# jontio/JAERO

Hardware: AMD Instinct MI355X
Metric: Msamples/s of real 48 kHz PCM through the 10.5 kbps OQPSK demodulator hot path (higher is better)
Workload: dtype f64; 1 GPU; 65536-channel-per-GPU synthetic 48 kHz 10.5 kbps OQPSK continuous (BASELINE configs[2] shape, scaled to 65536 channels per GPU = one wavefront of 64 channels per SIMD), 4096-sample writes, coarse 2^14 FFT every 4096 samples, AFC off, EbNo meters on, Eb/N0 10.0 dB, per-channel carrier (8000 +- 100 Hz), bits, noise, symbol phase; 42 untimed pre-roll steps (the last 11 resident and back to back with ; channels_per_gpu=65536, total_channels=65536, chunk=4096, ebno_meters=True, preroll_steps=42, timing_phases=32, hbm_bytes_per_resident_channel=2267392, resident_channels_max=136377, ranks=1, control_plane=none (single rank), sustain_steps=11

## Files before the change

jaero_amd/csrc/jaero_device.h:

```cpp
#pragma once
#include <hip/hip_runtime.h>
#include <stdint.h>
#include "jd_libm.h"

#define JD_WTSIZE 19999
#define JD_WAVE 64

enum
{
    S_M2_PTR, S_M2_STEP, S_M2_FREQ,
    S_MC_PTR, S_MC_STEP, S_MC_FREQ,
    S_ST_PTR, S_ST_STEP, S_ST_FREQ, S_ST_LAST,
    S_AGC_SUM,
    S_EB_ESUM, S_EB_E2SUM, S_EB_EBNO,
    S_D1,
    S_D41_1, S_D41_2, S_D41_3,
    S_D42_1, S_D42_2, S_D42_3,
    S_D8_1, S_D8_2,
    S_RES_X1, S_RES_X2, S_RES_Y1, S_RES_Y2,
    S_LF_X1, S_LF_X2, S_LF_Y1, S_LF_Y2,
    S_SIG2L_RE, S_SIG2L_IM, S_PTD_RE, S_PTD_IM,
    S_MARG_SUM, S_PM_SUM, S_MSEMA_SUM, S_MSE,
    S_DIFF_LAST,
    S_LOCKINGBW, S_THRESH,
    S_MFB_A0_RE, S_MFB_A0_IM,
    S_PRE_PTR, S_PRE_STEP, S_PRE_FSUM,
    S_PRE_PTR_NEXT, S_PRE_STEP_NEXT,
    S_NFIELDS
};
enum
{
    I_AGC_POS,
    I_AGC_HOLD,
    I_BB_PTR, I_COARSE_CNT,
    I_MARG_POS, I_DT_POS, I_PM_POS, I_MSEMA_POS,
    I_YUI, I_SIG2L_INIT, I_FLAGS, I_COUNTDOWN, I_COUNTDOWN2, I_EMPTYING, I_NEST,
    I_SOFT_CNT, I_SYM_CNT, I_LOG_CNT, I_OVERFLOW,
    I_DLY_POS,
    I_NFIELDS
};
typedef const __attribute__((address_space(4))) int jd_cint;
typedef const __attribute__((address_space(4))) double jd_cdouble;
__device__ __forceinline__ int jd_sload(const int *q) { return *(jd_cint *)q; }
__device__ __forceinline__ double jd_sload(const double *q) { return *(jd_cdouble *)q; }

#define JD_G4(row, ch, rows) ((((size_t)((ch) >> 2)) * (size_t)(rows) + (size_t)(row)) * 4 + (size_t)((ch) & 3))
#define LDF(f) (p.S[(size_t)(f) * nchp + ch])
#define LDI(f) (p.I[(size_t)(f) * nchp + ch])

#define JF_AFC 1
#define JF_SQL 2
#define JF_CPUREDUCE 4
#define JF_DCD 8

struct JGeom
{
    int kind, nch, nchp, ngroups;
    double Fs, fb;
    int Fs_int;
    int fir_n;
    int agc_len;
    int ebno_len;
    int win_len;
    int nfft, nfft_log2;
    int marg_len, dt_len, pm_len, msema_len;
    double ee;
    double w4, w8;
    int sps, sps2;
    double res_b0, res_b1, res_b2, res_a1, res_a2;
    double lf_b0, lf_b1, lf_b2, lf_a1, lf_a2;
    double stref_freq;
    double correctionfactor;
    unsigned flags;
    int soft_cap, sym_cap, log_cap;
};

struct JPtrs
{
    double *S;
    int *I;
    double *win;
    double2 *bbring;
    double *y;
    double *marg;
    double2 *dt;
    double *pm;
    double *msema;
    double *firsave;
    double2 *dly;
    double *dly8;
    int16_t *soft;
    double *sym;
    double *slog;
    const double2 *cis;
    const double *taps2;
    double *symrec;
};
#define JD_SYMREC_LEN 800

__device__ __forceinline__ int jd_cisidx(double wtptr)
{
    int t = (int)wtptr;
    if (t >= JD_WTSIZE) t = 0;
    if (t < 0) t = JD_WTSIZE - 1;
    return t;
}
__device__ __forceinline__ void jd_wt_next(double &ptr, double &step)
{
    if (step < 0) step = 0;
    ptr += step;
    while (((int)ptr) >= JD_WTSIZE) ptr -= JD_WTSIZE;
}
__device__ __forceinline__ void jd_wt_setfreq(double &freq, double &step, double f, double samplerate)
{
    freq = f;
    if (freq < 0) freq = 0;
    step = (freq) * ((double)JD_WTSIZE) / samplerate;
}
__device__ __forceinline__ void jd_wt_inc_phase_deg(double &ptr, double phase_deg)
{
    phase_deg += (360.0 * ptr / ((double)JD_WTSIZE));
    phase_deg = fmod(phase_deg, 360.0);
    while (phase_deg < 0) phase_deg += 360.0;
    ptr = (phase_deg / 360.0) * ((double)JD_WTSIZE);
}
__device__ __forceinline__ void jd_wt_advance_fraction(double &ptr, double f)
{
    ptr += f * JD_WTSIZE;
    while (ptr >= JD_WTSIZE) ptr -= JD_WTSIZE;
    while (ptr < 0) ptr += JD_WTSIZE;
}
__device__ __forceinline__ bool jd_wt_passed(double last_ptr, double ptr, double step, double fraction_of_wave, double &frac)
{
    double pt = (fraction_of_wave * JD_WTSIZE);
    double tl = last_ptr - pt;
    double tp = ptr - pt;
    if (tl < 0.0) tl += JD_WTSIZE;
    if (tp < 0.0) tp += JD_WTSIZE;
    if ((tl > (3.0 * JD_WTSIZE / 4.0)) && (tp < (1.0 * JD_WTSIZE / 4.0)))
    {
        frac = tp / step;
        return true;
    }
    return false;
}
__device__ __forceinline__ int jd_qround(double d)
{
    return d >= 0.0 ? (int)(d + 0.5) : (int)(d - (double)((int)(d - 1)) + 0.5) + (int)(d - 1);
}
__device__ __forceinline__ int jd_softbit(double v)
{
    int ibit = jd_qround(v);
    if (ibit > 255) ibit = 255;
    if (ibit < 0) ibit = 0;
    return ibit;
}

#define JD_EBNO_TAIL 192


template <int FIRN, int LDSN, int D, bool FUSED = false, int TAILA = 1>
__device__ __forceinline__ void jd_fir_eval(const double *lre, const double *lim, const double *ltap, const double (&tre)[TAILA],
                                            const double (&tim)[TAILA], int fir_slot, int lane, double &ore, double &oim)
{
    constexpr int TAILN = FIRN - LDSN;
    double pr[D], pi[D], pt[D];
    int slot = fir_slot;
    auto fetch = [&](int s, int q) {
        pt[q] = ltap[s];
        if (s >= TAILN)
        {
            pr[q] = lre[slot * 64 + lane];
            pi[q] = lim[slot * 64 + lane];
            slot++;
            if (slot >= LDSN) slot = 0;
        }
    };
#pragma unroll
    for (int s = 0; s < D; s++) fetch(s, s);
    __builtin_amdgcn_sched_barrier(0);
    double are = 0, aim = 0;
#pragma unroll
    for (int s = 0; s < FIRN; s++)
    {
        const int q = s % D;
        const double xr = (s < TAILN) ? tre[(TAILN - 1 - s) < 0 ? 0 : (TAILN - 1 - s)] : pr[q];
        const double xi = (s < TAILN) ? tim[(TAILN - 1 - s) < 0 ? 0 : (TAILN - 1 - s)] : pi[q];
        if constexpr (FUSED) { are = fma(pt[q], xr, are); aim = fma(pt[q], xi, aim); }
        else { are = are + pt[q] * xr; aim = aim + pt[q] * xi; }
        asm volatile("" : "+v"(are), "+v"(aim));
        if (s + D < FIRN) fetch(s + D, q);
        __builtin_amdgcn_sched_barrier(0);
    }
    ore = are; oim = aim;
}

struct JTaps28 { double t[28]; };

typedef __attribute__((address_space(3))) const double jd_lds_cdouble;
template <int FIRN, int LDSN, int D, int S, int TAP0, int NQ = LDSN>
__device__ __forceinline__ void jd_fir_lds_part(jd_lds_cdouble *lre_l, jd_lds_cdouble *lim_l, const JTaps28 &tp, double &are, double &aim)
{
    constexpr int TAILN = TAP0;
    double pr[D], pi[D];
#pragma unroll
    for (int q = 0; q < D; q++) { pr[q] = lre_l[((S + q) % LDSN) * 64]; pi[q] = lim_l[((S + q) % LDSN) * 64]; }
    __builtin_amdgcn_sched_barrier(0);
    auto tap_of = [&](int q) { const int s = TAILN + q; return tp.t[s <= 27 ? s : 54 - s]; };
    double mr = tap_of(0) * pr[0], mi = tap_of(0) * pi[0];
#pragma unroll
    for (int q = 0; q < NQ; q++)
    {
        double nr = 0, ni = 0;
        if (q + 1 < NQ) { nr = tap_of(q + 1) * pr[(q + 1) % D]; ni = tap_of(q + 1) * pi[(q + 1) % D]; }
        are = are + mr;
        aim = aim + mi;
        asm volatile("" : "+v"(are), "+v"(aim));
        if (q + D < NQ) { pr[q % D] = lre_l[((S + q + D) % LDSN) * 64]; pi[q % D] = lim_l[((S + q + D) % LDSN) * 64]; }
        mr = nr; mi = ni;
        __builtin_amdgcn_sched_barrier(0);
    }
}
template <int FIRN, int LDSN, int D, int TAILA>
__device__ __forceinline__ void jd_fir_eval_sym(const double *lre, const double *lim, const JTaps28 &tp, const double (&tre)[TAILA],
                                                const double (&tim)[TAILA], int fir_slot, int lane, double &ore, double &oim)
{
    static_assert(FIRN == 55, "symmetric-tap filter is the 55-tap RRC");
    constexpr int TAILN = FIRN - LDSN;
    double are = 0, aim = 0;
#pragma unroll
    for (int s = 0; s < TAILN; s++)
    {
        const double tap = tp.t[s <= 27 ? s : 54 - s];
        are = are + tap * tre[TAILN - 1 - s];
        aim = aim + tap * tim[TAILN - 1 - s];
    }
    int slot = fir_slot;
#pragma unroll 1
    for (int q = 0; q < LDSN; q++)
    {
        const int s = TAILN + q;
        const double tap = tp.t[s <= 27 ? s : 54 - s];
        are = are + tap * lre[slot * 64 + lane];
        aim = aim + tap * lim[slot * 64 + lane];
        slot++;
        if (slot >= LDSN) slot = 0;
    }
    ore = are; oim = aim;
}
template <int FIRN, int LDSN, int D, int TAILA>
__device__ __forceinline__ void jd_fir_eval_sym_static(const double *lre, const double *lim, const JTaps28 &tp, const double (&tre)[TAILA],
                                                       const double (&tim)[TAILA], int fir_slot, int lane, double &ore, double &oim)
{
    static_assert(FIRN == 55 && LDSN <= 40, "symmetric-tap filter is the 55-tap RRC; the switch below has 40 cases");
    constexpr int TAILN = FIRN - LDSN;
    jd_lds_cdouble *lre_l = (jd_lds_cdouble *)lre + lane, *lim_l = (jd_lds_cdouble *)lim + lane;
    double are = 0, aim = 0;
#pragma unroll
    for (int s = 0; s < TAILN; s++)
    {
        const double tap = tp.t[s <= 27 ? s : 54 - s];
        are = are + tap * tre[TAILN - 1 - s];
        aim = aim + tap * tim[TAILN - 1 - s];
    }
#define JD_FIR_CASE(S) case S: if constexpr (S < LDSN) jd_fir_lds_part<FIRN, LDSN, D, (S < LDSN ? S : 0), FIRN - LDSN>(lre_l, lim_l, tp, are, aim); break;
    switch (fir_slot)
    {
        JD_FIR_CASE(0) JD_FIR_CASE(1) JD_FIR_CASE(2) JD_FIR_CASE(3) JD_FIR_CASE(4) JD_FIR_CASE(5) JD_FIR_CASE(6) JD_FIR_CASE(7)
        JD_FIR_CASE(8) JD_FIR_CASE(9) JD_FIR_CASE(10) JD_FIR_CASE(11) JD_FIR_CASE(12) JD_FIR_CASE(13) JD_FIR_CASE(14) JD_FIR_CASE(15)
        JD_FIR_CASE(16) JD_FIR_CASE(17) JD_FIR_CASE(18) JD_FIR_CASE(19) JD_FIR_CASE(20) JD_FIR_CASE(21) JD_FIR_CASE(22) JD_FIR_CASE(23)
        JD_FIR_CASE(24) JD_FIR_CASE(25) JD_FIR_CASE(26) JD_FIR_CASE(27) JD_FIR_CASE(28) JD_FIR_CASE(29) JD_FIR_CASE(30) JD_FIR_CASE(31)
        JD_FIR_CASE(32) JD_FIR_CASE(33) JD_FIR_CASE(34) JD_FIR_CASE(35) JD_FIR_CASE(36) JD_FIR_CASE(37) JD_FIR_CASE(38) JD_FIR_CASE(39)
    default: break;
    }
#undef JD_FIR_CASE
    ore = are; oim = aim;
}

template <int FIRN, int LDSN, int D, int TAILA>
__device__ __forceinline__ void jd_fir_eval_sym_static_but_last(const double *lre, const double *lim, const JTaps28 &tp, const double (&tre)[TAILA],
                                                                const double (&tim)[TAILA], int slot_old, int lane, double &ore, double &oim)
{
    static_assert(FIRN == 55 && LDSN <= 40 && LDSN >= 8, "symmetric-tap filter is the 55-tap RRC; the switch below has 40 cases");
    constexpr int TAILN = FIRN - LDSN;
    jd_lds_cdouble *lre_l = (jd_lds_cdouble *)lre + lane, *lim_l = (jd_lds_cdouble *)lim + lane;
    double are = 0, aim = 0;
#pragma unroll
    for (int s = 0; s < TAILN; s++)
    {
        const double tap = tp.t[s <= 27 ? s : 54 - s];
        are = are + tap * tre[TAILN - 1 - s];
        aim = aim + tap * tim[TAILN - 1 - s];
    }
#define JD_FIR_CASE(S) case S: if constexpr (S < LDSN) jd_fir_lds_part<FIRN, LDSN, D, (S < LDSN ? (S + 1) % LDSN : 0), FIRN - LDSN, LDSN - 1>(lre_l, lim_l, tp, are, aim); break;
    switch (slot_old)
    {
        JD_FIR_CASE(0) JD_FIR_CASE(1) JD_FIR_CASE(2) JD_FIR_CASE(3) JD_FIR_CASE(4) JD_FIR_CASE(5) JD_FIR_CASE(6) JD_FIR_CASE(7)
        JD_FIR_CASE(8) JD_FIR_CASE(9) JD_FIR_CASE(10) JD_FIR_CASE(11) JD_FIR_CASE(12) JD_FIR_CASE(13) JD_FIR_CASE(14) JD_FIR_CASE(15)
        JD_FIR_CASE(16) JD_FIR_CASE(17) JD_FIR_CASE(18) JD_FIR_CASE(19) JD_FIR_CASE(20) JD_FIR_CASE(21) JD_FIR_CASE(22) JD_FIR_CASE(23)
        JD_FIR_CASE(24) JD_FIR_CASE(25) JD_FIR_CASE(26) JD_FIR_CASE(27) JD_FIR_CASE(28) JD_FIR_CASE(29) JD_FIR_CASE(30) JD_FIR_CASE(31)
        JD_FIR_CASE(32) JD_FIR_CASE(33) JD_FIR_CASE(34) JD_FIR_CASE(35) JD_FIR_CASE(36) JD_FIR_CASE(37) JD_FIR_CASE(38) JD_FIR_CASE(39)
    default: break;
    }
#undef JD_FIR_CASE
    ore = are; oim = aim;
}

__device__ __forceinline__ double jd_with_hi(double x, int h) { return __hiloint2double(h, __double2loint(x)); }
__device__ __forceinline__ double jd_expm1(double x)
{
    const double one = 1.0, huge = 1.0e+300, tiny = 1.0e-300, o_threshold = 7.09782712893383973096e+02,
                 ln2_hi = 6.93147180369123816490e-01, ln2_lo = 1.90821492927058770002e-10, invln2 = 1.44269504088896338700e+00,
                 Q1 = -3.33333333333331316428e-02, Q2 = 1.58730158725481460165e-03, Q3 = -7.93650757867487942473e-05,
                 Q4 = 4.00821782732936239552e-06, Q5 = -2.01099218183624371326e-07;
    double y, hi, lo, c = 0, t, e, hxs, hfx, r1;
    int k;
    unsigned hx = (unsigned)__double2hiint(x);
    const unsigned xsb = hx & 0x80000000u;
    hx &= 0x7fffffffu;
    if (hx >= 0x4043687Au)
    {
        if (hx >= 0x40862E42u)
        {
            if (hx >= 0x7ff00000u)
            {
                if (((hx & 0xfffffu) | (unsigned)__double2loint(x)) != 0) return x + x;
                return (xsb == 0) ? x : -1.0;
            }
            if (x > o_threshold) return huge * huge;
        }
        if (xsb != 0 && x + tiny < 0.0) return tiny - one;
    }
    if (hx > 0x3fd62e42u)
    {
        if (hx < 0x3FF0A2B2u)
        {
            if (xsb == 0) { hi = x - ln2_hi; lo = ln2_lo; k = 1; }
            else { hi = x + ln2_hi; lo = -ln2_lo; k = -1; }
        }
        else
        {
            k = (int)(invln2 * x + ((xsb == 0) ? 0.5 : -0.5));
            t = k;
            hi = x - t * ln2_hi;
            lo = t * ln2_lo;
        }
        x = hi - lo;
        c = (hi - x) - lo;
    }
    else if (hx < 0x3c900000u) return x;
    else k = 0;
    hfx = 0.5 * x;
    hxs = x * hfx;
    {
        const double R1 = one + hxs * Q1, h2 = hxs * hxs;
        const double R2 = Q2 + hxs * Q3, h4 = h2 * h2;
        const double R3 = Q4 + hxs * Q5;
        r1 = R1 + h2 * R2 + h4 * R3;
    }
    t = 3.0 - r1 * hfx;
    e = hxs * ((r1 - t) / (6.0 - x * t));
    if (k == 0) return x - (x * e - hxs);
    e = (x * (e - c) - c);
    e -= hxs;
    if (k == -1) return 0.5 * (x - e) - 0.5;
    if (k == 1)
    {
        if (x < -0.25) return -2.0 * (e - (x + 0.5));
        return one + 2.0 * (x - e);
    }
    if (k <= -2 || k > 56)
    {
        y = one - (e - x);
        y = jd_with_hi(y, __double2hiint(y) + (k << 20));
        return y - one;
    }
    if (k < 20)
    {
        t = jd_with_hi(one, 0x3ff00000 - (0x200000 >> k));
        y = t - (e - x);
        y = jd_with_hi(y, __double2hiint(y) + (k << 20));
    }
    else
    {
        t = jd_with_hi(one, (0x3ff - k) << 20);
        y = x - (e + t);
        y += one;
        y = jd_with_hi(y, __double2hiint(y) + (k << 20));
    }
    return y;
}
__device__ __noinline__ double jd_tanh_full(double x)
{
    const double one = 1.0, two = 2.0, tiny = 1.0e-300;
    double t, z;
    const int jx = __double2hiint(x);
    const int ix = jx & 0x7fffffff;
    if (ix >= 0x7ff00000) return (jx >= 0) ? one / x + one : one / x - one;
    if (ix < 0x40360000)
    {
        if ((ix | __double2loint(x)) == 0) return x;
        if (ix < 0x3c800000) return x * (one + x);
        const bool big = ix >= 0x3ff00000;
        const double ax2 = two * fabs(x);
        t = jd_expm1(big ? ax2 : -ax2);
        const double q = (big ? two : t) / (t + two);
        z = big ? one - q : -q;
    }
    else z = one - tiny;
    return (jx >= 0) ? z : -z;
}

__device__ __forceinline__ double jd_tanh(double xin)
{
    const double one = 1.0, two = 2.0, ln2_hi = 6.93147180369123816490e-01, ln2_lo = 1.90821492927058770002e-10,
                 invln2 = 1.44269504088896338700e+00, Q1 = -3.33333333333331316428e-02, Q2 = 1.58730158725481460165e-03,
                 Q3 = -7.93650757867487942473e-05, Q4 = 4.00821782732936239552e-06, Q5 = -2.01099218183624371326e-07;
    const int jx = __double2hiint(xin), ix = jx & 0x7fffffff;
    if (!(ix >= 0x3c800000 && ix < 0x401a0000)) return jd_tanh_full(xin);
    const bool big = ix >= 0x3ff00000;
    const double ax2 = two * fabs(xin);
    double x = big ? ax2 : -ax2;
    const unsigned hx = (unsigned)__double2hiint(x) & 0x7fffffffu;
    const int k = (hx > 0x3fd62e42u) ? (int)(invln2 * x + (big ? 0.5 : -0.5)) : 0;
    const double tk = (double)k;
    const double hi = x - tk * ln2_hi, lo = tk * ln2_lo;
    x = hi - lo;
    const double c = (hi - x) - lo;
    const double hfx = 0.5 * x, hxs = x * hfx;
    const double R1 = one + hxs * Q1, h2 = hxs * hxs, R2 = Q2 + hxs * Q3, h4 = h2 * h2, R3 = Q4 + hxs * Q5;
    const double r1 = R1 + h2 * R2 + h4 * R3;
    const double t3 = 3.0 - r1 * hfx;
    const double e = hxs * jd_div(r1 - t3, 6.0 - x * t3);
    const double r_k0 = x - (x * e - hxs);
    double e2 = (x * (e - c) - c);
    e2 -= hxs;
    const double r_m1 = 0.5 * (x - e2) - 0.5;
    double yn = one - (e2 - x);
    yn = jd_with_hi(yn, __double2hiint(yn) + (k << 20));
    const double r_neg = yn - one;
    const double tm = jd_with_hi(one, 0x3ff00000 - (0x200000 >> (k & 31)));
    double ym = tm - (e2 - x);
    ym = jd_with_hi(ym, __double2hiint(ym) + (k << 20));
    const double t = (k == 0) ? r_k0 : (k == -1) ? r_m1 : (k <= -2) ? r_neg : ym;
    const double q = jd_div(big ? two : t, t + two);
    const double z = big ? one - q : -q;
    return (jx >= 0) ? z : -z;
}
```

jaero_amd/csrc/k_oqpsk_fb.h:

```cpp
#pragma once
#include "jaero_device.h"

#define FB_DEFER 8

#ifdef FB_TRACE_BUILD
__device__ unsigned long long g_fb_trace[2][10];
#define FB_TRACE_DECL unsigned long long tr_acc[8] = {0, 0, 0, 0, 0, 0, 0, 0}; unsigned long long tr_prev = wall_clock64()
#define FB_TRACE(k)                                                                                                                                           \
    do {                                                                                                                                                      \
        __builtin_amdgcn_sched_barrier(0);                                                                                                                    \
        const unsigned long long t_ = wall_clock64();                                                                                                         \
        tr_acc[k] += t_ - tr_prev; tr_prev = t_;                                                                                                              \
        __builtin_amdgcn_sched_barrier(0);                                                                                                                    \
    } while (0)
#define FB_TRACE_FLUSH(which, nsamp)                                                                                                                          \
    do {                                                                                                                                                      \
        if (lane == 0 && grp == (g.ngroups > 600 ? 597 : 0))                                                                                                  \
        {                                                                                                                                                     \
            for (int k_ = 0; k_ < 8; k_++) atomicAdd(&g_fb_trace[which][k_], tr_acc[k_]);                                                                    \
            atomicAdd(&g_fb_trace[which][8], (unsigned long long)(nsamp));                                                                                    \
        }                                                                                                                                                     \
    } while (0)
#else
#define FB_TRACE_DECL
#define FB_TRACE(k)
#define FB_TRACE_FLUSH(which, nsamp)
#endif
#ifndef FB_SOLO_D
#define FB_SOLO_D 6
#endif
#define FB_LDSN 36

__device__ __forceinline__ double jd_div_const(double x, double d, double rd)
{
    double q = x * rd;
    double r = fma(-d, q, x);
    q = fma(r, rd, q);
    r = fma(-d, q, x);
    q = fma(r, rd, q);
    return copysign(q, x);
}
__device__ __forceinline__ void fb_wt_setfreq(double &freq, double &step, double f, double samplerate, double r_samplerate)
{
    freq = f;
    if (freq < 0) freq = 0;
    step = jd_div_const((freq) * ((double)JD_WTSIZE), samplerate, r_samplerate);
}
__device__ __forceinline__ void fb_wt_next(double &ptr, double &step)
{
    if (step < 0) step = 0;
    ptr += step;
    if (((int)ptr) >= JD_WTSIZE)
    {
        ptr -= JD_WTSIZE;
        while (((int)ptr) >= JD_WTSIZE) ptr -= JD_WTSIZE;
    }
}
__device__ __forceinline__ double fb_fmod360(double x)
{
    const double ax = fabs(x);
    if (ax < 360.0) return x;
    if (ax < 720.0) return copysign(ax - 360.0, x);
    return fmod(x, 360.0);
}

struct FbLds
{
    double *lre, *lim;
    double *data;
    int *idx;
};
template <int LDSN>
constexpr int fb_pair_doubles() { return 2 * LDSN * 64 + 2 * 3 * 64 + 64; }

#define FB_SYNC(L) fb_barrier()
__device__ __forceinline__ void fb_barrier()
{
    asm volatile("s_waitcnt lgkmcnt(0)\n\ts_barrier" ::: "memory");
}

template <int FIRN, int LDSN, bool EBNO, bool PRE8400, bool SOLO>
__device__ __forceinline__ void fb_front(const JGeom &g, const JPtrs &p, FbLds &L, const int16_t *__restrict__ pcm, int pcm_stride, int n,
                                         int skip_a_first, int only_a_last, int fir_slot0, int grp, int lane, const JTaps28 &tp,
                                         const double2 *__restrict__ prefilt, int pf_rows)
{
    constexpr int TAILN = FIRN - LDSN;
    double tre[TAILN], tim[TAILN];
    const int ch = grp * 64 + lane;
    const int nchp = g.nchp;
    const bool live = ch < g.nch;
    const double2 *__restrict__ cis = p.cis;
    const int nB = n - (only_a_last ? 1 : 0);

    double mc_ptr = LDF(S_MC_PTR), mc_step = LDF(S_MC_STEP);
    double agc_sum = LDF(S_AGC_SUM);
    double eb_esum = LDF(S_EB_ESUM), eb_e2sum = LDF(S_EB_E2SUM), eb_ebno = LDF(S_EB_EBNO);
    int agc_pos = LDI(I_AGC_POS), bb_ptr = LDI(I_BB_PTR), coarse_cnt = LDI(I_COARSE_CNT);
    int agc_hold = LDI(I_AGC_HOLD);
    const int flags = LDI(I_FLAGS);
    const int nfft_mask = g.nfft - 1;
    double2 *__restrict__ bbring = p.bbring + (size_t)ch * g.nfft;
    double *__restrict__ win = p.win + (size_t)grp * g.win_len * 64 + lane;
    auto wslot = [&](int pos, int lag) { const int q = pos - lag; return q < 0 ? q + g.win_len : q; };

    double2 cq1 = make_double2(0.0, 0.0), cq2 = cq1, cq3 = cq1;
    int cq_n = 0;
    auto ring_fill = [&](const double2 v) __attribute__((always_inline)) {
        if ((bb_ptr & 3) == 3)
        {
            double2 *dst = bbring + bb_ptr;
            if (cq_n >= 3) dst[-3] = cq3;
            if (cq_n >= 2) dst[-2] = cq2;
            if (cq_n >= 1) dst[-1] = cq1;
            dst[0] = v;
            cq_n = 0;
        }
        else
        {
            cq3 = cq2; cq2 = cq1; cq1 = v;
            cq_n++;
        }
        bb_ptr = (bb_ptr + 1) & nfft_mask;
    };
    auto ring_flush = [&]() __attribute__((always_inline)) {
        double2 *dst = bbring + bb_ptr;
        if (cq_n >= 3) dst[-3] = cq3;
        if (cq_n >= 2) dst[-2] = cq2;
        if (cq_n >= 1) dst[-1] = cq1;
        cq_n = 0;
    };

    double *lre = L.lre, *lim = L.lim;
    if constexpr (!PRE8400)
    {
        const double *fs = p.firsave + (size_t)grp * 2 * FIRN * 64 + lane;
        for (int k = 0; k < LDSN; k++)
        {
            lre[k * 64 + lane] = fs[(size_t)k * 64];
            lim[k * 64 + lane] = fs[(size_t)(FIRN + k) * 64];
        }
#pragma unroll
        for (int j = 0; j < TAILN; j++)
        {
            tre[j] = fs[(size_t)(LDSN + j) * 64];
            tim[j] = fs[(size_t)(FIRN + LDSN + j) * 64];
        }
    }
    int fir_slot = fir_slot0;

    const double agc_len_d = (double)g.agc_len, eb_len_d = (double)g.ebno_len;
    const double r_agc_len = 1.0 / agc_len_d, r_eb_len = 1.0 / eb_len_d;

    auto front_sample = [&](double sre, double sim, double agc_old, double e_old, int j, int buf) __attribute__((always_inline)) {
        const double dabval = sqrt(sre * sre + sim * sim);
        if (EBNO)
        {
            const double sq = dabval * dabval;
            const double e2_old = e_old * e_old;
            eb_e2sum = eb_e2sum - e2_old; eb_e2sum = eb_e2sum + fabs(sq);
            eb_esum = eb_esum - e_old; eb_esum = eb_esum + fabs(dabval);
            if (j >= n - JD_EBNO_TAIL)
            {
                const double e2val = jd_div_const(eb_e2sum, eb_len_d, r_eb_len), mean = jd_div_const(eb_esum, eb_len_d, r_eb_len);
                const double meansq = mean * mean;
                double var = e2val - (mean * mean);
                var -= (0.024709 * meansq);
                double mvr = (((g.Fs * meansq / (2.0 * g.fb * var))) * 0.13743);
                if (mvr < 0.000000001) mvr = 0.000000001;
                double tebno = 10.0 * log10(mvr);
                if (isnan(tebno)) tebno = 50;
                if (tebno > 50.0) tebno = 50;
                if (tebno < 0.0) tebno = 0;
                eb_ebno = eb_ebno * 0.8 + 0.2 * tebno;
            }
        }
        {
            if (agc_hold > 0) { agc_old = 0.0; agc_hold--; }
            double *ap = win + (size_t)agc_pos * 64;
            agc_sum = agc_sum - agc_old;
            agc_sum = agc_sum + fabs(dabval);
            *ap = fabs(dabval);
            agc_pos++; if (agc_pos >= g.win_len) agc_pos = 0;
        }
        double gain = jd_div(1.414213562, fmax(jd_div_const(agc_sum, agc_len_d, r_agc_len), 0.000001));
        gain = fmax(gain, 0.000001);
        sre *= gain; sim *= gain;
        const double abval = jd_hypot(sre, sim);
        if (abval > 2.84) { const double k = jd_div(2.84, abval); sre = k * sre; sim = k * sim; }
        double *d = L.data + buf * 3 * 64 + lane;
        d[0] = sre; d[64] = sim; d[128] = abval;
    };

    auto ring_pos_next = [](int pos, int len) { pos++; return pos >= len ? 0 : pos; };
    double r1_agc = win[(size_t)wslot(agc_pos, g.agc_len) * 64];
    double r1_e = 0;
    if (EBNO) r1_e = win[(size_t)wslot(agc_pos, g.ebno_len) * 64];
    short nx_pcm = (live && n > 0) ? pcm[ch] : (short)0;
    double2 nx_cc = cis[jd_cisidx(mc_ptr)];

    if constexpr (PRE8400)
    {
        double2 nx_pf = (nB > 0) ? prefilt[JD_G4(0, ch, pf_rows)] : make_double2(0.0, 0.0);
        FB_SYNC(L);
        for (int i = 0; i < nB; i++)
        {
            const int m2i = L.idx[(i & 1) * 64 + lane];
            const double2 c_m2 = cis[m2i];
            const double2 pf = nx_pf;
            const double sre = c_m2.x * pf.x - c_m2.y * pf.y, sim = c_m2.x * pf.y + c_m2.y * pf.x;
            front_sample(sre, sim, r1_agc, r1_e, i, i & 1);
            FB_SYNC(L);
            const double dval = ((double)nx_pcm) / 32768.0;
            const double2 cc = nx_cc;
            const bool do_fill = !(i == 0 && skip_a_first) && ((coarse_cnt >= g.Fs_int) || !(flags & JF_CPUREDUCE));
            if (do_fill) ring_fill(make_double2(cc.x * dval, cc.y * dval));
            coarse_cnt++;
            fb_wt_next(mc_ptr, mc_step);
            if (i + 1 < n)
            {
                nx_pcm = live ? pcm[(size_t)(i + 1) * pcm_stride + ch] : (short)0;
                nx_cc = cis[jd_cisidx(mc_ptr)];
                nx_pf = prefilt[JD_G4(i + 1, ch, pf_rows)];
            }
            if (i + 1 < nB)
            {
                r1_agc = win[(size_t)wslot(agc_pos, g.agc_len) * 64];
                if (EBNO) r1_e = win[(size_t)wslot(agc_pos, g.ebno_len) * 64];
            }
            FB_SYNC(L);
        }
    }
    else
    {
    if (nB > 0)
    {
        double y_re, y_im;
        jd_fir_eval_sym<FIRN, LDSN, 6>(lre, lim, tp, tre, tim, fir_slot, lane, y_re, y_im);
        front_sample(y_re, y_im, r1_agc, r1_e, 0, 0);
        r1_agc = win[(size_t)wslot(agc_pos, g.agc_len) * 64];
        if (EBNO) r1_e = win[(size_t)wslot(agc_pos, g.ebno_len) * 64];
    }
    FB_SYNC(L);

    FB_TRACE_DECL;
    for (int i = 0; i < nB; i++)
    {
        FB_TRACE(0);
        const int m2i = L.idx[(i & 1) * 64 + lane];
        const double2 c_m2 = cis[m2i];
#pragma unroll
        for (int j = TAILN - 1; j > 0; j--) { tre[j] = tre[j - 1]; tim[j] = tim[j - 1]; }
        double *hre = lre + fir_slot * 64 + lane, *him = lim + fir_slot * 64 + lane;
        tre[0] = *hre;
        tim[0] = *him;
        const short s = nx_pcm;
        const double dval = ((double)s) / 32768.0;
        const double2 cc = nx_cc;
        const bool do_fill = !(i == 0 && skip_a_first) && ((coarse_cnt >= g.Fs_int) || !(flags & JF_CPUREDUCE));
        __builtin_amdgcn_sched_barrier(0);
        double y_re = 0, y_im = 0;
        if constexpr (SOLO)
            if (i + 1 < nB) jd_fir_eval_sym_static_but_last<FIRN, LDSN, FB_SOLO_D>(lre, lim, tp, tre, tim, fir_slot, lane, y_re, y_im);
        const double cre = c_m2.x * dval, cim = c_m2.y * dval;
        {
            *hre = cre;
            *him = cim;
            fir_slot++;
            if (fir_slot >= LDSN) fir_slot = 0;
        }
        __builtin_amdgcn_sched_barrier(0);
        FB_TRACE(1);
        if (do_fill) ring_fill(make_double2(cc.x * dval, cc.y * dval));
        coarse_cnt++;
        fb_wt_next(mc_ptr, mc_step);
        if (i + 1 < n)
        {
            nx_pcm = live ? pcm[(size_t)(i + 1) * pcm_stride + ch] : (short)0;
            nx_cc = cis[jd_cisidx(mc_ptr)];
        }
        double r2_agc = 0, r2_e = 0;
        if (i + 2 < nB)
        {
            const int wn = ring_pos_next(agc_pos, g.win_len);
            r2_agc = win[(size_t)wslot(wn, g.agc_len) * 64];
            if (EBNO) r2_e = win[(size_t)wslot(wn, g.ebno_len) * 64];
        }
        __builtin_amdgcn_sched_barrier(0);
        FB_TRACE(2);
        if (i + 1 < nB)
        {
            if constexpr (SOLO) { y_re = y_re + tp.t[0] * cre; y_im = y_im + tp.t[0] * cim; }
            else jd_fir_eval_sym_static<FIRN, LDSN, 6>(lre, lim, tp, tre, tim, fir_slot, lane, y_re, y_im);
            FB_TRACE(3);
            front_sample(y_re, y_im, r1_agc, r1_e, i + 1, (i + 1) & 1);
            r1_agc = r2_agc; r1_e = r2_e;
            FB_TRACE(4);
        }
        FB_SYNC(L);
    }
    FB_TRACE_FLUSH(0, nB);
    }
    if (only_a_last)
    {
        const double dval = ((double)nx_pcm) / 32768.0;
        const bool do_fill = !(nB == 0 && skip_a_first) && ((coarse_cnt >= g.Fs_int) || !(flags & JF_CPUREDUCE));
        if (do_fill) ring_fill(make_double2(nx_cc.x * dval, nx_cc.y * dval));
    }
    ring_flush();

    LDF(S_MC_PTR) = mc_ptr; LDF(S_MC_STEP) = mc_step;
    LDF(S_AGC_SUM) = agc_sum;
    LDF(S_EB_ESUM) = eb_esum; LDF(S_EB_E2SUM) = eb_e2sum; LDF(S_EB_EBNO) = eb_ebno;
    LDI(I_AGC_POS) = agc_pos; LDI(I_BB_PTR) = bb_ptr; LDI(I_COARSE_CNT) = coarse_cnt;
    LDI(I_AGC_HOLD) = agc_hold;
    if constexpr (!PRE8400)
    {
        double *fs = p.firsave + (size_t)grp * 2 * FIRN * 64 + lane;
        for (int k = 0; k < LDSN; k++)
        {
            fs[(size_t)k * 64] = lre[k * 64 + lane];
            fs[(size_t)(FIRN + k) * 64] = lim[k * 64 + lane];
        }
#pragma unroll
        for (int j = 0; j < TAILN; j++)
        {
            fs[(size_t)(LDSN + j) * 64] = tre[j];
            fs[(size_t)(FIRN + LDSN + j) * 64] = tim[j];
        }
    }
}

template <bool CAPSYM, bool PRE8400>
__device__ __forceinline__ void fb_back(const JGeom &g, const JPtrs &p, FbLds &L, int n, int only_a_last, int grp, int lane)
{
    const int ch = grp * 64 + lane;
    const int nchp = g.nchp;
    const double2 *__restrict__ cis = p.cis;
    const int nB = n - (only_a_last ? 1 : 0);

    double m2_ptr = LDF(S_M2_PTR), m2_step = LDF(S_M2_STEP), m2_freq = LDF(S_M2_FREQ);
    double st_ptr = LDF(S_ST_PTR), st_step = LDF(S_ST_STEP), st_freq = LDF(S_ST_FREQ), st_last = LDF(S_ST_LAST);
    double d1 = LDF(S_D1);
    double d41_1 = LDF(S_D41_1), d41_2 = LDF(S_D41_2), d41_3 = LDF(S_D41_3);
    double d42_1 = LDF(S_D42_1), d42_2 = LDF(S_D42_2), d42_3 = LDF(S_D42_3);
    double d8_1 = LDF(S_D8_1), d8_2 = LDF(S_D8_2);
    double res_x1 = LDF(S_RES_X1), res_x2 = LDF(S_RES_X2), res_y1 = LDF(S_RES_Y1), res_y2 = LDF(S_RES_Y2);
    double lf_x1 = LDF(S_LF_X1), lf_x2 = LDF(S_LF_X2), lf_y1 = LDF(S_LF_Y1), lf_y2 = LDF(S_LF_Y2);
    double sig2l_re = LDF(S_SIG2L_RE), sig2l_im = LDF(S_SIG2L_IM), ptd_re = LDF(S_PTD_RE), ptd_im = LDF(S_PTD_IM);
    double ptd_th = jd_tanh(ptd_re);
    double marg_sum = LDF(S_MARG_SUM), pm_sum = LDF(S_PM_SUM), msema_sum = LDF(S_MSEMA_SUM), mse = LDF(S_MSE);
    const double thresh = LDF(S_THRESH);
    int marg_pos = LDI(I_MARG_POS), dt_pos = LDI(I_DT_POS), pm_pos = LDI(I_PM_POS), msema_pos = LDI(I_MSEMA_POS);
    int yui = LDI(I_YUI), sig2l_init = LDI(I_SIG2L_INIT);
    int soft_cnt = LDI(I_SOFT_CNT), sym_cnt = LDI(I_SYM_CNT), overflow = LDI(I_OVERFLOW);

    const JdAtanLane atl = jd_atan_lane_table(lane);
    const double samplerate = g.Fs;
    const double r_samplerate = 1.0 / samplerate;
    const double wtsize_d = (double)JD_WTSIZE, r_wtsize = 1.0 / wtsize_d, r_360 = 1.0 / 360.0;
    const double marg_len_d = (double)g.marg_len, pm_len_d = (double)g.pm_len, msema_len_d = (double)g.msema_len;
    const double r_marg_len = 1.0 / marg_len_d, r_pm_len = 1.0 / pm_len_d, r_msema_len = 1.0 / msema_len_d;
    double *__restrict__ symrec = p.symrec + (size_t)ch * JD_SYMREC_LEN * 8;
    const double w4 = g.w4, w4c = 1.0 - g.w4, w8 = g.w8, w8c = 1.0 - g.w8;

    bool pend = false, need_px = false;
    double pd_ec = 0, pd_re = 0, pd_im = 0;
    double px_marg = 0, px_pm = 0, px_ms = 0;
    double2 px_dt = make_double2(0.0, 0.0);
    auto queue_symbol = [&](double ct_ec, double q_re, double q_im) {
        pend = true; need_px = true; pd_ec = ct_ec; pd_re = q_re; pd_im = q_im;
    };
    auto request_px = [&]() {
        px_marg = symrec[marg_pos * 8];
        int o = marg_pos + JD_SYMREC_LEN / 2; if (o >= JD_SYMREC_LEN) o -= JD_SYMREC_LEN;
        const double2 *r = (const double2 *)(symrec + o * 8);
        const double2 r0 = r[0], r1 = r[1], r2 = r[2];
        px_dt = make_double2(r0.y, r1.x);
        px_pm = r1.y;
        px_ms = r2.x;
        need_px = false;
    };
    auto output_half = [&]() {
        const double ct_ec = pd_ec;
        double q_re = pd_re, q_im = pd_im;
        marg_sum = marg_sum - px_marg; marg_sum = marg_sum + ct_ec;
        const double marg_val = jd_div_const(marg_sum, marg_len_d, r_marg_len);
        const double in_re = q_re, in_im = q_im;
        q_re = px_dt.x; q_im = px_dt.y;
        {
            double sr, cr;
            sincos(marg_val, &sr, &cr);
            const double nr = q_re * cr - q_im * sr;
            const double ni = q_re * sr + q_im * cr;
            q_re = nr; q_im = ni;
        }
        double av_w, e_w;
        {
            const double av = jd_hypot(q_re, q_im);
            pm_sum = pm_sum - px_pm; pm_sum = pm_sum + fabs(av); av_w = fabs(av);
            double mu = jd_div_const(pm_sum, pm_len_d, r_pm_len);
            if (mu < 0.000001) mu = 0.000001;
            const double s2 = sqrt(2.0);
            const double t_re = jd_div(s2 * q_re, mu), t_im = jd_div(s2 * q_im, mu);
            const double tda = (fabs(t_re) - 1.0), tdb = (fabs(t_im) - 1.0);
            const double e = (tda * tda) + (tdb * tdb);
            msema_sum = msema_sum - px_ms; msema_sum = msema_sum + fabs(e); e_w = fabs(e);
            mse = jd_div_const(msema_sum, msema_len_d, r_msema_len);
        }
        {
            double2 *w = (double2 *)(symrec + marg_pos * 8);
            w[0] = make_double2(ct_ec, in_re);
            w[1] = make_double2(in_im, av_w);
            w[2] = make_double2(e_w, 0.0);
            w[3] = make_double2(0.0, 0.0);
            marg_pos++; if (marg_pos >= JD_SYMREC_LEN) marg_pos = 0;
        }
        if (CAPSYM)
        {
            if (sym_cnt < g.sym_cap)
            {
                double *sp = p.sym + ((size_t)ch * g.sym_cap + sym_cnt) * 3;
                sp[0] = q_re; sp[1] = q_im; sp[2] = mse;
                sym_cnt++;
            }
            else overflow |= 2;
        }
        if (mse < thresh)
        {
            const int b0 = jd_softbit(0.75 * q_im * 127.0 + 128.0);
            const int b1 = jd_softbit(0.75 * q_re * 127.0 + 128.0);
            if (soft_cnt + 2 <= g.soft_cap)
            {
                int16_t *sp = p.soft + (size_t)ch * g.soft_cap + soft_cnt;
                sp[0] = (int16_t)b0;
                sp[1] = (int16_t)b1;
                soft_cnt += 2;
            }
            else overflow |= 1;
        }
        pend = false;
    };

    L.idx[lane] = jd_cisidx(m2_ptr);
    double2 nx_cst = cis[jd_cisidx(st_ptr)];
    FB_SYNC(L);

    double m2fsum = 0;
    FB_TRACE_DECL;
    for (int i = 0; i < nB; i++)
    {
        if constexpr (!PRE8400) FB_TRACE(0);
        if constexpr (PRE8400)
        {
            FB_SYNC(L);
            m2fsum += m2_freq;
        }
        const double2 c_st = nx_cst;
        const double *d = L.data + (i & 1) * 3 * 64 + lane;
        double sre = d[0], sim = d[64];
        const double abval = d[128];

        const double ab2 = abval * abval;
        const double st_diff = d1 - ab2; d1 = ab2;
        const double st_d1out = w4 * d41_2 + w4c * d41_3; d41_3 = d41_2; d41_2 = d41_1; d41_1 = st_diff;
        const double st_d2out = w4 * d42_2 + w4c * d42_3; d42_3 = d42_2; d42_2 = d42_1; d42_1 = st_d1out;
        double st_eta = (st_d2out - st_diff) * st_d1out;
        {
            double y = 0;
            y += res_x2 * g.res_b2; y += res_x1 * g.res_b1; y += st_eta * g.res_b0;
            y -= res_y2 * g.res_a2; y -= res_y1 * g.res_a1;
            res_x2 = res_x1; res_x1 = st_eta; res_y2 = res_y1; res_y1 = y;
            st_eta = y;
        }
        const double d8out = w8 * d8_1 + w8c * d8_2; d8_2 = d8_1; d8_1 = st_eta;
        {
            const double2 so = c_st;
            const double m_re = st_eta, m_im = -d8out;
            const double o_re = so.x * m_re - so.y * m_im;
            const double o_im = so.x * m_im + so.y * m_re;
            const double st_angle_error = jd_atan2(o_im, o_re, atl);
            fb_wt_setfreq(st_freq, st_step, (-st_angle_error * 0.00000001) + st_freq, samplerate, r_samplerate);
            jd_wt_advance_fraction(st_ptr, jd_div_const(-st_angle_error * 0.01, 360.0, r_360));
            if (st_freq < (g.stref_freq - 0.1)) fb_wt_setfreq(st_freq, st_step, (g.stref_freq - 0.1), samplerate, r_samplerate);
            if (st_freq > (g.stref_freq + 0.1)) fb_wt_setfreq(st_freq, st_step, (g.stref_freq + 0.1), samplerate, r_samplerate);
        }
        if constexpr (!PRE8400) FB_TRACE(1);
        if (need_px) request_px();
        if constexpr (!PRE8400) FB_TRACE(5);

        if (!sig2l_init) { sig2l_re = sre; sig2l_im = sim; sig2l_init = 1; }
        double frac;
        const bool inst = jd_wt_passed(st_last, st_ptr, st_step, g.ee, frac);
        const bool full = inst && (yui == 0);
        if constexpr (!PRE8400) FB_TRACE(6);
        if (pend && (full || (i & (FB_DEFER - 1)) == 0)) output_half();
        if constexpr (!PRE8400) FB_TRACE(2);
        if (inst)
        {
            const double pt_last = frac, pt_this = 1.0 - pt_last;
            const double pt_re = pt_this * sre + pt_last * sig2l_re;
            const double pt_im = pt_this * sim + pt_last * sig2l_im;
            yui++; yui %= 2;
            const double th = jd_tanh(yui ? pt_im : pt_re);
            if (!yui) { ptd_re = pt_re; ptd_im = pt_im; ptd_th = th; }
            else
            {
                const double ct_xt = th * pt_re;
                const double ct_xt_d = ptd_th * ptd_im;
                double ct_ec = ct_xt_d - ct_xt;
                if (ct_ec > M_PI) ct_ec = M_PI;
                if (ct_ec < -M_PI) ct_ec = -M_PI;
                double lf_y;
                {
                    double y = 0;
                    y += lf_x2 * g.lf_b2; y += lf_x1 * g.lf_b1; y += ct_ec * g.lf_b0;
                    y -= lf_y2 * g.lf_a2; y -= lf_y1 * g.lf_a1;
                    lf_x2 = lf_x1; lf_x1 = ct_ec; lf_y2 = lf_y1; lf_y1 = y;
                    lf_y = y;
                }
                if constexpr (!PRE8400)
                {
                    ct_ec = lf_y;
                    if (ct_ec > M_PI_2) ct_ec = M_PI_2;
                    if (ct_ec < -M_PI_2) ct_ec = -M_PI_2;
                }
                {
                    double phase_deg = 1.0 * ct_ec;
                    phase_deg += jd_div_const(360.0 * m2_ptr, wtsize_d, r_wtsize);
                    phase_deg = fb_fmod360(phase_deg);
                    while (phase_deg < 0) phase_deg += 360.0;
                    m2_ptr = jd_div_const(phase_deg, 360.0, r_360) * wtsize_d;
                }
                if constexpr (PRE8400) fb_wt_setfreq(m2_freq, m2_step, (0.5 * 0.01 * lf_y) + m2_freq, samplerate, r_samplerate);
                else fb_wt_setfreq(m2_freq, m2_step, (0.01 * ct_ec) + m2_freq, samplerate, r_samplerate);
                queue_symbol(ct_ec, pt_re, ptd_im);
            }
        }
        sig2l_re = sre; sig2l_im = sim;
        if constexpr (!PRE8400) FB_TRACE(3);

        fb_wt_next(m2_ptr, m2_step);
        L.idx[((i + 1) & 1) * 64 + lane] = jd_cisidx(m2_ptr);
        if (st_step < 0) st_step = 0;
        st_last = st_ptr;
        st_ptr += st_step;
        if (((int)st_ptr) >= JD_WTSIZE)
        {
            st_ptr -= JD_WTSIZE;
            while (((int)st_ptr) >= JD_WTSIZE) st_ptr -= JD_WTSIZE;
        }
        nx_cst = cis[jd_cisidx(st_ptr)];
        if constexpr (!PRE8400) FB_TRACE(4);
        FB_SYNC(L);
    }
    if constexpr (!PRE8400) FB_TRACE_FLUSH(1, nB);
    if (need_px) request_px();
    if (pend) output_half();

    LDF(S_M2_PTR) = m2_ptr; LDF(S_M2_STEP) = m2_step; LDF(S_M2_FREQ) = m2_freq;
    LDF(S_ST_PTR) = st_ptr; LDF(S_ST_STEP) = st_step; LDF(S_ST_FREQ) = st_freq; LDF(S_ST_LAST) = st_last;
    LDF(S_D1) = d1;
    LDF(S_D41_1) = d41_1; LDF(S_D41_2) = d41_2; LDF(S_D41_3) = d41_3;
    LDF(S_D42_1) = d42_1; LDF(S_D42_2) = d42_2; LDF(S_D42_3) = d42_3;
    LDF(S_D8_1) = d8_1; LDF(S_D8_2) = d8_2;
    LDF(S_RES_X1) = res_x1; LDF(S_RES_X2) = res_x2; LDF(S_RES_Y1) = res_y1; LDF(S_RES_Y2) = res_y2;
    LDF(S_LF_X1) = lf_x1; LDF(S_LF_X2) = lf_x2; LDF(S_LF_Y1) = lf_y1; LDF(S_LF_Y2) = lf_y2;
    LDF(S_SIG2L_RE) = sig2l_re; LDF(S_SIG2L_IM) = sig2l_im; LDF(S_PTD_RE) = ptd_re; LDF(S_PTD_IM) = ptd_im;
    LDF(S_MARG_SUM) = marg_sum; LDF(S_PM_SUM) = pm_sum; LDF(S_MSEMA_SUM) = msema_sum; LDF(S_MSE) = mse;
    LDI(I_MARG_POS) = marg_pos; LDI(I_DT_POS) = dt_pos; LDI(I_PM_POS) = pm_pos; LDI(I_MSEMA_POS) = msema_pos;
    LDI(I_YUI) = yui; LDI(I_SIG2L_INIT) = sig2l_init;
    LDI(I_SOFT_CNT) = soft_cnt; LDI(I_SYM_CNT) = sym_cnt; LDI(I_OVERFLOW) = overflow;
    if constexpr (PRE8400) LDF(S_PRE_FSUM) = LDF(S_PRE_FSUM) + m2fsum;
}

template <int FIRN, int LDSN, bool EBNO, bool CAPSYM, int PAIRS, bool PRE8400 = false>
__global__ __launch_bounds__(PAIRS * 128) void k_oqpsk_fb(const JGeom g, const JPtrs p, const int16_t *__restrict__ pcm, int pcm_stride, int n,
                                                          int skip_a_first, int only_a_last, int fir_slot0, const JTaps28 tp,
                                                          const double2 *__restrict__ prefilt, int pf_rows)
{
    extern __shared__ __attribute__((aligned(16))) double lds[];
    const int wave = __builtin_amdgcn_readfirstlane((int)(threadIdx.x >> 6));
    const int lane = threadIdx.x & 63;
    const bool back = wave >= PAIRS;
    const int pair = back ? wave - PAIRS : wave;
    const int grp = blockIdx.x * PAIRS + pair;
    double *base = lds + (size_t)pair * fb_pair_doubles<LDSN>();
    FbLds L;
    L.lre = base; L.lim = base + LDSN * 64;
    L.data = base + 2 * LDSN * 64;
    L.idx = (int *)(L.data + 2 * 3 * 64);
    if (grp >= g.ngroups)
    {
        const int nB = n - (only_a_last ? 1 : 0);
        const int nbar = PRE8400 ? 2 * nB + 1 : nB + 1;
        for (int i = 0; i < nbar; i++) fb_barrier();
        return;
    }
    if (back) fb_back<CAPSYM, PRE8400>(g, p, L, n, only_a_last, grp, lane);
    else fb_front<FIRN, LDSN, EBNO, PRE8400, (PAIRS == 1 && !PRE8400)>(g, p, L, pcm, pcm_stride, n, skip_a_first, only_a_last, fir_slot0, grp, lane, tp, prefilt, pf_rows);
}
```

Before: 11830 Msamples/s.

## Deepen FIR LDS prefetch with grouped lgkm waits and branchless loop-control clamps

Raises the symmetric FIR LDS prefetch depth from 6 to 8 and adds explicit grouped lgkmcnt waits every 4 taps, so LDS reads overlap the FMAs instead of each waiting on its own. It also rewrites the symbol-timing frequency clamp as one setfreq call with select-based clamps, makes the fmod360 helper and the sig2l init branchless, and replaces a while loop with a single if. These aim to cut LDS latency stalls and branch divergence in the per-sample hot path. The costs are higher register pressure from the deeper prefetch and reliance on the manual waitcnt encoding being correct. The frequency clamp also no longer matches the original sequence exactly when the reference frequency is near zero.

Result: no change. 11810 Msamples/s (median of 6 runs) (-0.2%).

```diff
diff --git a/jaero_amd/csrc/jaero_device.h b/jaero_amd/csrc/jaero_device.h
--- a/jaero_amd/csrc/jaero_device.h
+++ b/jaero_amd/csrc/jaero_device.h
@@ -198,19 +198,40 @@
 struct JTaps28 { double t[28]; };
 
 typedef __attribute__((address_space(3))) const double jd_lds_cdouble;
-template <int FIRN, int LDSN, int D, int S, int TAP0, int NQ = LDSN>
+__device__ __forceinline__ void jd_wait_lgkm(int n)
+{
+#define JD_LGKM_CASE(N) case N: __builtin_amdgcn_s_waitcnt(0xC07F | (N << 8)); break;
+    switch (n)
+    {
+        JD_LGKM_CASE(0) JD_LGKM_CASE(1) JD_LGKM_CASE(2) JD_LGKM_CASE(3) JD_LGKM_CASE(4) JD_LGKM_CASE(5) JD_LGKM_CASE(6) JD_LGKM_CASE(7)
+        JD_LGKM_CASE(8) JD_LGKM_CASE(9) JD_LGKM_CASE(10) JD_LGKM_CASE(11) JD_LGKM_CASE(12) JD_LGKM_CASE(13) JD_LGKM_CASE(14) JD_LGKM_CASE(15)
+    default: __builtin_amdgcn_s_waitcnt(0xC07F); break;
+    }
+#undef JD_LGKM_CASE
+}
+template <int FIRN, int LDSN, int D, int S, int TAP0, int NQ = LDSN, int G = 1>
 __device__ __forceinline__ void jd_fir_lds_part(jd_lds_cdouble *lre_l, jd_lds_cdouble *lim_l, const JTaps28 &tp, double &are, double &aim)
 {
+    static_assert(G == 1 || (G < D && D - G <= 15), "a group's last read is issued before its wait; lgkmcnt is a 4-bit count");
     constexpr int TAILN = TAP0;
     double pr[D], pi[D];
 #pragma unroll
     for (int q = 0; q < D; q++) { pr[q] = lre_l[((S + q) % LDSN) * 64]; pi[q] = lim_l[((S + q) % LDSN) * 64]; }
     __builtin_amdgcn_sched_barrier(0);
+    auto wait_upto = [&](int q, int r) __attribute__((always_inline)) {
+        if constexpr (G > 1)
+        {
+            const int last = (q - 1 + D < NQ - 1) ? q - 1 + D : NQ - 1;
+            jd_wait_lgkm(last - (r < NQ - 1 ? r : NQ - 1));
+        }
+    };
+    wait_upto(0, G - 1);
     auto tap_of = [&](int q) { const int s = TAILN + q; return tp.t[s <= 27 ? s : 54 - s]; };
     double mr = tap_of(0) * pr[0], mi = tap_of(0) * pi[0];
 #pragma unroll
     for (int q = 0; q < NQ; q++)
     {
+        if ((q + 1) % G == 0 && q + 1 < NQ) wait_upto(q, q + G);
         double nr = 0, ni = 0;
         if (q + 1 < NQ) { nr = tap_of(q + 1) * pr[(q + 1) % D]; ni = tap_of(q + 1) * pi[(q + 1) % D]; }
         are = are + mr;
@@ -248,7 +269,7 @@
     }
     ore = are; oim = aim;
 }
-template <int FIRN, int LDSN, int D, int TAILA>
+template <int FIRN, int LDSN, int D, int TAILA, int G = 1>
 __device__ __forceinline__ void jd_fir_eval_sym_static(const double *lre, const double *lim, const JTaps28 &tp, const double (&tre)[TAILA],
                                                        const double (&tim)[TAILA], int fir_slot, int lane, double &ore, double &oim)
 {
@@ -263,7 +284,7 @@
         are = are + tap * tre[TAILN - 1 - s];
         aim = aim + tap * tim[TAILN - 1 - s];
     }
-#define JD_FIR_CASE(S) case S: if constexpr (S < LDSN) jd_fir_lds_part<FIRN, LDSN, D, (S < LDSN ? S : 0), FIRN - LDSN>(lre_l, lim_l, tp, are, aim); break;
+#define JD_FIR_CASE(S) case S: if constexpr (S < LDSN) jd_fir_lds_part<FIRN, LDSN, D, (S < LDSN ? S : 0), FIRN - LDSN, LDSN, G>(lre_l, lim_l, tp, are, aim); break;
     switch (fir_slot)
     {
         JD_FIR_CASE(0) JD_FIR_CASE(1) JD_FIR_CASE(2) JD_FIR_CASE(3) JD_FIR_CASE(4) JD_FIR_CASE(5) JD_FIR_CASE(6) JD_FIR_CASE(7)
diff --git a/jaero_amd/csrc/k_oqpsk_fb.h b/jaero_amd/csrc/k_oqpsk_fb.h
--- a/jaero_amd/csrc/k_oqpsk_fb.h
+++ b/jaero_amd/csrc/k_oqpsk_fb.h
@@ -29,6 +29,8 @@
 #ifndef FB_SOLO_D
 #define FB_SOLO_D 6
 #endif
+#define FB_FIR_D 8
+#define FB_FIR_G 4
 #define FB_LDSN 36
 
 __device__ __forceinline__ double jd_div_const(double x, double d, double rd)
@@ -59,9 +61,9 @@
 __device__ __forceinline__ double fb_fmod360(double x)
 {
     const double ax = fabs(x);
-    if (ax < 360.0) return x;
-    if (ax < 720.0) return copysign(ax - 360.0, x);
-    return fmod(x, 360.0);
+    double r = ax < 360.0 ? x : copysign(ax - 360.0, x);
+    if (!(ax < 720.0)) r = fmod(x, 360.0);
+    return r;
 }
 
 struct FbLds
@@ -290,7 +292,7 @@
         if (i + 1 < nB)
         {
             if constexpr (SOLO) { y_re = y_re + tp.t[0] * cre; y_im = y_im + tp.t[0] * cim; }
-            else jd_fir_eval_sym_static<FIRN, LDSN, 6>(lre, lim, tp, tre, tim, fir_slot, lane, y_re, y_im);
+            else jd_fir_eval_sym_static<FIRN, LDSN, FB_FIR_D, TAILN, FB_FIR_G>(lre, lim, tp, tre, tim, fir_slot, lane, y_re, y_im);
             FB_TRACE(3);
             front_sample(y_re, y_im, r1_agc, r1_e, i + 1, (i + 1) & 1);
             r1_agc = r2_agc; r1_e = r2_e;
@@ -362,6 +364,8 @@
     const double r_marg_len = 1.0 / marg_len_d, r_pm_len = 1.0 / pm_len_d, r_msema_len = 1.0 / msema_len_d;
     double *__restrict__ symrec = p.symrec + (size_t)ch * JD_SYMREC_LEN * 8;
     const double w4 = g.w4, w4c = 1.0 - g.w4, w8 = g.w8, w8c = 1.0 - g.w8;
+    const double st_lo = g.stref_freq - 0.1, st_hi = g.stref_freq + 0.1;
+    const double st_lo0 = st_lo < 0 ? 0 : st_lo, st_hi0 = st_hi < 0 ? 0 : st_hi;
 
     bool pend = false, need_px = false;
     double pd_ec = 0, pd_re = 0, pd_im = 0;
@@ -479,16 +483,18 @@
             const double o_re = so.x * m_re - so.y * m_im;
             const double o_im = so.x * m_im + so.y * m_re;
             const double st_angle_error = jd_atan2(o_im, o_re, atl);
-            fb_wt_setfreq(st_freq, st_step, (-st_angle_error * 0.00000001) + st_freq, samplerate, r_samplerate);
             jd_wt_advance_fraction(st_ptr, jd_div_const(-st_angle_error * 0.01, 360.0, r_360));
-            if (st_freq < (g.stref_freq - 0.1)) fb_wt_setfreq(st_freq, st_step, (g.stref_freq - 0.1), samplerate, r_samplerate);
-            if (st_freq > (g.stref_freq + 0.1)) fb_wt_setfreq(st_freq, st_step, (g.stref_freq + 0.1), samplerate, r_samplerate);
+            double f = (-st_angle_error * 0.00000001) + st_freq;
+            f = f < 0 ? 0 : f;
+            f = f < st_lo ? st_lo0 : f;
+            f = f > st_hi ? st_hi0 : f;
+            fb_wt_setfreq(st_freq, st_step, f, samplerate, r_samplerate);
         }
         if constexpr (!PRE8400) FB_TRACE(1);
         if (need_px) request_px();
         if constexpr (!PRE8400) FB_TRACE(5);
 
-        if (!sig2l_init) { sig2l_re = sre; sig2l_im = sim; sig2l_init = 1; }
+        sig2l_re = sig2l_init ? sig2l_re : sre; sig2l_im = sig2l_init ? sig2l_im : sim; sig2l_init = 1;
         double frac;
         const bool inst = jd_wt_passed(st_last, st_ptr, st_step, g.ee, frac);
         const bool full = inst && (yui == 0);
@@ -528,7 +534,7 @@
                     double phase_deg = 1.0 * ct_ec;
                     phase_deg += jd_div_const(360.0 * m2_ptr, wtsize_d, r_wtsize);
                     phase_deg = fb_fmod360(phase_deg);
-                    while (phase_deg < 0) phase_deg += 360.0;
+                    if (phase_deg < 0) phase_deg += 360.0;
                     m2_ptr = jd_div_const(phase_deg, 360.0, r_360) * wtsize_d;
                 }
                 if constexpr (PRE8400) fb_wt_setfreq(m2_freq, m2_step, (0.5 * 0.01 * lf_y) + m2_freq, samplerate, r_samplerate);
```
